# pnnl/nmrfit

Measured on NVIDIA B200. Metric: voigt_objective_evals_per_s, higher is better.
Workload: dtype f64

## Files before the change

### nmrfit_b200/csrc/cabi.cu

```cuda
#include <cuda_runtime.h>
#include <algorithm>
#include <cmath>
#include <atomic>
#include <cstdio>
#include <cstdlib>
#include <cstring>
#include <new>
#include <string>
#include <vector>
#include "../../include/nmrfit_b200.h"
#include "nmrfit_internal.h"

namespace nmrfit {
std::atomic<long long> g_launches{0};
void count_launches(int n) { g_launches.fetch_add(n, std::memory_order_relaxed); }
}

using namespace nmrfit;

namespace {

thread_local std::string t_error;

int fail(int code, const std::string& msg) {
    t_error = msg;
    return code;
}

int fail_cuda(cudaError_t e, const char* where) {
    t_error = std::string(where) + ": " + cudaGetErrorName(e) + " (" + cudaGetErrorString(e) + ")";
    return NMRFIT_ERR_CUDA;
}

#define CK(call)                                              \
    do {                                                      \
        cudaError_t _e = (call);                              \
        if (_e != cudaSuccess) return fail_cuda(_e, #call);   \
    } while (0)

template <typename T>
struct DevBuf {
    T* ptr = nullptr;
    size_t cap = 0;
    cudaError_t reserve(size_t n) {
        if (n <= cap) return cudaSuccess;
        if (ptr) cudaFree(ptr);
        ptr = nullptr;
        cap = 0;
        cudaError_t e = cudaMalloc(&ptr, n * sizeof(T));
        if (e == cudaSuccess) cap = n;
        return e;
    }
    void release() {
        if (ptr) cudaFree(ptr);
        ptr = nullptr;
        cap = 0;
    }
};

bool is_device_pointer(const void* p) {
    cudaPointerAttributes at;
    if (cudaPointerGetAttributes(&at, p) != cudaSuccess) {
        cudaGetLastError();
        return false;
    }
    return at.type == cudaMemoryTypeDevice || at.type == cudaMemoryTypeManaged;
}

}

constexpr int kShadowSpectra = 4;

struct nmrfit_ctx {
    int device = 0, B = 0, N = 0, P = 0, D = 0, precision = 0;
    DevBuf<double> spec;
    std::vector<char> spec_set;
    std::vector<std::vector<double>> shadow;
    DevBuf<double> grid_h;
    std::vector<char> uniform;
    int algorithm = NMRFIT_ALGO_AUTO;
    DevBuf<double> partials, x_stage, f_stage;
    DevBuf<double> prep_coef, prep_part, prep_far, prep_anchor;
    DevBuf<unsigned> prep_mask;
    ObjTune user_tune{0, 0, 0, 0, -1, 0, 0};
    bool swarm = false;
    SwarmState sw{};
    int maxiter = 0, kk = 0, generation = 0;
    DevBuf<double> sx, sv, sp, sfx, sfp, sg, sfg, sbx, sbf, slb, sub, srec, rnd_a, rnd_b;
    DevBuf<int> sstop, sit;
    DevBuf<double> frec_f, frec_x;
    DevBuf<unsigned> fbarrier;
    DevBuf<int> ferror;
    DevBuf<unsigned> mt_state;
    DevBuf<unsigned> mt_words;
    long long mt_elems = 0;
    DevBuf<double> mt_a[2], mt_b[2];
    DevBuf<unsigned> mt_state2, mt_words2;
    cudaStream_t mt_stream = nullptr;
    unsigned* mt_host = nullptr;
    int mt_flip = 0, mt_pending = 0;
    DevBuf<double> fin_scratch;
    DevBuf<unsigned> fin_tickets;
    void* peer_win = nullptr;
    size_t peer_rec_bytes = 0;
    int peer_ranks = 0, peer_rank = 0;
    bool peers_ready = false;
    std::vector<void*> peer_opened;
    DevBuf<double*> peer_recs_dev;
    DevBuf<long long*> peer_tok_dev;
    DevBuf<int> peer_err;
    long long epoch = 0;
    double peer_timeout_ms = 20000.0;
    DevBuf<double> wscratch, wbounds;
    cudaStream_t pipe[2] = {nullptr, nullptr};
    double* h_f = nullptr;
    size_t h_f_cap = 0;
    int far_cells = 0;
    int fused_mode = NMRFIT_FUSED_AUTO;
    DevBuf<long long> ftiming;
    bool fused_timing = false;
    long long fused_launches = 0;
    int* h_flags = nullptr;
    bool profiling = false;
    std::vector<cudaEvent_t> prof_events;
    size_t prof_used = 0;
};

struct nmrfit_phase {
    int device = 0, B = 0, N = 0;
    DevBuf<double> u, v, cands, out;
    DevBuf<int> ok;
};

struct nmrfit_peaks {
    int device = 0, B = 0, N = 0, upsample = 100, max_peaks = 0;
    long long M = 0;
    int nblk = 0;
    DevBuf<double> w, u, uu, us, bmax, base, uu_at, pk_h, sg;
    DevBuf<long long> maxima, pk_i, cross, probe_idx;
    DevBuf<int> n_maxima, n_pk;
    DevBuf<char> out;
    DevBuf<double> probe_out;
    bool ran = false;
};

namespace {

bool axis_is_uniform(const double* hw, int N, double* grid) {
    double h = 0.0, big = 0.0;
    bool uni = N >= 2;
    if (uni) {
        h = (hw[N - 1] - hw[0]) / (double)(N - 1);
        big = std::max(std::fabs(hw[0]), std::fabs(hw[N - 1]));
        const double tol = 4.0 * 2.220446049250313e-16 * big;
        uni = std::isfinite(h) && h != 0.0 && std::isfinite(big);
        for (int i = 0; uni && i < N; ++i) uni = std::fabs(hw[i] - std::fma((double)i, h, hw[0])) <= tol;
    }
    grid[0] = h;
    grid[1] = 2.220446049250313e-16 * big;
    return uni;
}

bool use_uniform(const nmrfit_ctx* c, int fit_im) {
    if (c->algorithm == NMRFIT_ALGO_GENERAL) return false;
    if (fit_im == NMRFIT_IM_SUM || (fit_im == NMRFIT_IM_REFERENCE && c->precision != NMRFIT_FP64)) return false;
    for (char u : c->uniform)
        if (!u) return false;
    return true;
}

int ctx_cells(const nmrfit_ctx* c, int r) { return c->far_cells ? c->far_cells : far_cells_per_region(c->N, r); }

ObjTune pick_tune(const nmrfit_ctx* c, int S, bool uni) {
    ObjTune t;
    if (uni) {
        if (c->N >= 2048) { t.threads = 256; t.r = 8; }
        else { t.threads = 128; t.r = 4; }
    } else {
        if (c->N >= 8192) { t.threads = 256; t.r = 4; }
        else if (c->N >= 1024) { t.threads = 128; t.r = 4; }
        else { t.threads = 128; t.r = 2; }
    }
    t.tb = 6;
    if (c->user_tune.threads) t.threads = c->user_tune.threads;
    if (c->user_tune.r) t.r = c->user_tune.r;
    if (c->user_tune.tb == -1) t.tb = 0;
    else if (c->user_tune.tb > 0) t.tb = c->user_tune.tb;
    int n_tiles = (c->N + t.threads * t.r - 1) / (t.threads * t.r);
    long long ctas1 = (long long)n_tiles * S * c->B;
    int sp = (int)std::max<long long>(1, std::min<long long>(16, ctas1 / (148 * 4)));
    sp = std::min(sp, std::max(1, S));
    if (c->user_tune.sp > 0) sp = std::min(c->user_tune.sp, std::max(1, S));
    t.sp = sp;
    t.variant = 0;
    t.stages = 0;
    t.occ = 3;
    const long long particle_tiles = (long long)((c->N + t.threads * t.r - 1) / (t.threads * t.r)) * S * c->B;
    const bool enough = particle_tiles >= 8192 || c->user_tune.variant == 1;
    if (uni && c->precision == NMRFIT_FP64 && c->user_tune.variant != 0 && t.tb == 6 && enough) {
        t.variant = 1;
        t.occ = c->user_tune.occ == 3 ? 3 : 2;
        const size_t budget = (t.occ == 2 ? 112 : 74) * 1024;
        auto fit_sp = [&](int stg) {
            t.stages = stg;
            int spg = 0;
            for (int cand = 1; cand <= 16; ++cand) {
                t.sp = cand;
                if (objective_stream_smem_bytes(c->P, t, ctx_cells(c, t.r)) <= budget) spg = cand;
            }
            return spg;
        };
        int stg = c->user_tune.stages > 0 ? c->user_tune.stages : 3;
        int spg = fit_sp(stg);
        if (c->user_tune.stages == 0 && spg < 6) {
            const int spg2 = fit_sp(2);
            if (spg2 > spg) { stg = 2; spg = spg2; }
        }
        t.stages = stg;
        t.sp = std::max(1, spg);
        bool fits = true;
        if (c->user_tune.sp > 0) {
            t.sp = c->user_tune.sp;
            if (objective_stream_smem_bytes(c->P, t, ctx_cells(c, t.r)) > 200 * 1024 && c->user_tune.stages == 0) t.stages = 2;
            fits = objective_stream_smem_bytes(c->P, t, ctx_cells(c, t.r)) <= 200 * 1024;
        }
        if (fits) {
            t.sp = std::min(t.sp, std::max(1, S));
            return t;
        }
        t.variant = 0;
        t.stages = 0;
        t.occ = 3;
    }
    const bool f32 = c->precision == NMRFIT_FP32;
    auto uni_bytes = [&]() { return f32 ? objective_f32_smem_bytes(c->P, t) : objective_uniform_smem_bytes(c->P, t, ctx_cells(c, t.r)); };
    while (t.sp > 1 && (uni ? uni_bytes() : objective_smem_bytes(c->P, t, 2)) > 200 * 1024)
        t.sp /= 2;
    if (uni && c->user_tune.sp <= 0)
        while (t.sp > 4 && uni_bytes() > 74 * 1024) t.sp -= 1;
    return t;
}

int check_ctx(const nmrfit_ctx* c) {
    if (!c) return fail(NMRFIT_ERR_ARG, "ctx is NULL");
    return NMRFIT_OK;
}

int run_objective(nmrfit_ctx* c, const double* x_dev, int S, int fit_im, double* f_dev, const int* frozen,
                  cudaStream_t st, const MoveArgs* mv = nullptr, int* tiles_out = nullptr, int* nsum_out = nullptr,
                  int* nw_out = nullptr, size_t slot0 = 0, size_t slots_total = 0, const double* x_in = nullptr) {
    for (int b = 0; b < c->B; ++b)
        if (!c->spec_set[b]) return fail(NMRFIT_ERR_STATE, "spectrum " + std::to_string(b) + " was never set");
    if (fit_im < 0 || fit_im > 2) return fail(NMRFIT_ERR_ARG, "fit_im must be 0, 1 or 2");
    const bool uni = use_uniform(c, fit_im);
    if (c->algorithm == NMRFIT_ALGO_UNIFORM && !uni)
        return fail(NMRFIT_ERR_STATE, "the uniform-axis kernel needs uniformly spaced w in every spectrum and fit_im off");
    if (c->precision == NMRFIT_FP32 && fit_im != NMRFIT_REAL_ONLY)
        return fail(NMRFIT_ERR_ARG, "fit_im is not available in FP32 mode (the Kramers-Kronig term runs in FP64 only)");
    ObjTune t = pick_tune(c, S, uni);
    if (uni && c->precision == NMRFIT_FP32 && t.r == 16) t.r = 8;
    if (uni ? (t.r != 4 && t.r != 8 && t.r != 16) : (t.r != 2 && t.r != 4 && t.r != 8))
        return fail(NMRFIT_ERR_ARG, uni ? "points_per_thread must be 4, 8 or 16 for the uniform-axis kernel"
                                        : "points_per_thread must be 2, 4 or 8 for the general kernel");
    int n_tiles = objective_tiles(c->N, t);
    const size_t part_per = (size_t)n_tiles * 2 * (t.variant == 1 ? t.threads / 32 : 1);
    CK(c->partials.reserve(std::max((size_t)c->B * S, slots_total) * part_per));
    ObjArgs a{};
    const int sub = (uni && c->precision == NMRFIT_FP64) ? ctx_cells(c, t.r) : 1;
    if (uni) {
        size_t nc, np, nf, na, nm;
        int pad = 0;
        objective_uniform_prep_sizes(c->N, c->P, t, sub, &nc, &np, &nf, &na, &nm, &pad);
        const size_t slots = std::max((size_t)c->B * S, slots_total) + pad;
        CK(c->prep_coef.reserve(slots * nc));
        CK(c->prep_part.reserve(slots * np));
        CK(c->prep_far.reserve(slots * nf));
        CK(c->prep_anchor.reserve(slots * na));
        CK(c->prep_mask.reserve(slots * nm));
        a.prep_coef = c->prep_coef.ptr + slot0 * nc; a.prep_part = c->prep_part.ptr + slot0 * np;
        a.prep_far = c->prep_far.ptr + slot0 * nf; a.prep_anchor = c->prep_anchor.ptr + slot0 * na;
        a.prep_mask = c->prep_mask.ptr + slot0 * nm;
    }
    a.spec = c->spec.ptr;
    a.x = x_dev;
    a.x_in = x_in;
    a.partials = c->partials.ptr + slot0 * part_per;
    a.frozen = frozen;
    a.grid_h = c->grid_h.ptr;
    a.N = c->N; a.P = c->P; a.S = S; a.kk = fit_im; a.sp = t.sp; a.sub = sub;
    cudaEvent_t ev0 = nullptr, evm = nullptr, ev1 = nullptr;
    if (c->profiling) {
        if (c->prof_used + 3 > c->prof_events.size()) {
            for (int k = 0; k < 3; ++k) {
                cudaEvent_t ev;
                CK(cudaEventCreate(&ev));
                c->prof_events.push_back(ev);
            }
        }
        ev0 = c->prof_events[c->prof_used];
        evm = c->prof_events[c->prof_used + 1];
        ev1 = c->prof_events[c->prof_used + 2];
        c->prof_used += 3;
    }
    const bool two_pass = uni && c->precision == NMRFIT_FP64;
    if (evm && !two_pass) {
        CK(cudaEventRecord(ev0, st));
        CK(cudaEventRecord(evm, st));
        ev0 = nullptr;
    }
    const bool move_in_prepare = mv && uni && c->precision == NMRFIT_FP64;
    if (mv && !move_in_prepare) {
        cudaError_t em = launch_swarm_move(mv->s, mv->rp, mv->rg, mv->generation, st);
        if (em != cudaSuccess) return fail_cuda(em, "swarm move");
    }
    if (nsum_out) *nsum_out = c->precision == NMRFIT_FP32 ? 1 : (fit_im ? 2 : 1);
    if (nw_out) *nw_out = 1;
    cudaError_t e = c->precision == NMRFIT_FP32 ? launch_objective_f32(a, t, c->B, f_dev, uni, st, ev0, ev1, tiles_out)
                    : uni ? launch_objective_uniform(a, t, c->B, f_dev, st, ev0, ev1, move_in_prepare ? mv : nullptr, tiles_out, evm, nw_out)
                          : launch_objective(a, t, c->B, f_dev, st, ev0, ev1, tiles_out);
    if (e != cudaSuccess) return fail_cuda(e, "objective launch");
    return NMRFIT_OK;
}

int stage(const double* src, size_t n, DevBuf<double>& buf, cudaStream_t st, const double** out) {
    if (!src) { *out = nullptr; return NMRFIT_OK; }
    if (is_device_pointer(src)) { *out = src; return NMRFIT_OK; }
    CK(buf.reserve(n));
    CK(cudaMemcpyAsync(buf.ptr, src, n * sizeof(double), cudaMemcpyHostToDevice, st));
    *out = buf.ptr;
    return NMRFIT_OK;
}

int fused_setup(nmrfit_ctx* c, int n_gen, const double* rp_d, const double* rg_d, FusedArgs* a, FusedPlan* plan) {
    plan->ok = false;
    if (c->fused_mode == NMRFIT_FUSED_OFF) return NMRFIT_OK;
    if (c->precision != NMRFIT_FP64 || c->kk != NMRFIT_REAL_ONLY || !use_uniform(c, NMRFIT_REAL_ONLY)) return NMRFIT_OK;
    const SwarmState& s = c->sw;
    ObjTune t = pick_tune(c, s.S, true);
    *a = FusedArgs{};
    a->s = s;
    a->spec = c->spec.ptr;
    a->grid_h = c->grid_h.ptr;
    a->rp = rp_d;
    a->rg = rg_d;
    a->N = c->N; a->P = c->P;
    a->n_vtiles = objective_tiles(c->N, t);
    a->vw = t.threads / 32;
    a->sub = ctx_cells(c, t.r);
    a->n_gen = n_gen;
    a->gen0 = c->generation + 1;
    a->maxiter = c->maxiter;
    cudaError_t e = swarm_fused_plan(*a, c->D, s.B, s.S, t, c->device, c->fused_mode == NMRFIT_FUSED_REQUIRE, plan);
    if (e != cudaSuccess) return fail_cuda(e, "fused swarm plan");
    if (!plan->ok) return NMRFIT_OK;
    CK(c->frec_f.reserve(2 * (size_t)s.B * s.S));
    CK(c->frec_x.reserve(2 * (size_t)s.B * s.S * s.D));
    CK(c->fbarrier.reserve(s.B));
    if (!c->ferror.ptr) {
        CK(c->ferror.reserve(1));
        CK(cudaMemset(c->ferror.ptr, 0, sizeof(int)));
    }
    a->error = c->ferror.ptr;
    a->max_wait_ns = 10LL * 1000 * 1000 * 1000;
    a->rec_f = c->frec_f.ptr;
    a->rec_x = c->frec_x.ptr;
    a->barrier = c->fbarrier.ptr;
    a->timing = c->fused_timing ? c->ftiming.ptr : nullptr;
    return NMRFIT_OK;
}

PeerArgs make_peer_args(const nmrfit_ctx* c) {
    PeerArgs pa{};
    pa.recs = c->peer_recs_dev.ptr;
    pa.tokens = c->peer_tok_dev.ptr;
    pa.n_ranks = c->peer_ranks;
    pa.rank = c->peer_rank;
    pa.token = (c->epoch << 32) | (long long)c->generation;
    pa.max_wait_ns = (long long)(c->peer_timeout_ms * 1e6);
    pa.error = c->peer_err.ptr;
    return pa;
}

int swarm_generation(nmrfit_ctx* c, bool move, const double* rp_d, const double* rg_d, int commit, cudaStream_t st) {
    SwarmState& s = c->sw;
    if (commit == 2 && !c->peers_ready) return fail(NMRFIT_ERR_STATE, "nmrfit_pso_peer_open has not been called");
    const PeerArgs pa = commit == 2 ? make_peer_args(c) : PeerArgs{};
    MoveArgs mv{s, rp_d, rg_d, c->generation};
    int n_tiles = 0, nsum = 1, nw = 1;
    if (int rc = run_objective(c, s.x, s.S, c->kk, nullptr, move ? s.stop : nullptr, st, move ? &mv : nullptr, &n_tiles, &nsum,
                               &nw))
        return rc;
    cudaError_t e = launch_swarm_finish(s, c->partials.ptr, n_tiles, nsum, c->N, s.rec, c->fin_scratch.ptr,
                                        c->fin_tickets.ptr, commit, c->maxiter, st, nw, commit == 2 ? &pa : nullptr);
    if (e != cudaSuccess) return fail_cuda(e, "swarm finish");
    return NMRFIT_OK;
}

}

extern "C" {

int nmrfit_abi_version(void) { return NMRFIT_ABI_VERSION; }

const char* nmrfit_last_error(void) { return t_error.c_str(); }

int nmrfit_device_count(int* count) {
    if (!count) return fail(NMRFIT_ERR_ARG, "count is NULL");
    CK(cudaGetDeviceCount(count));
    return NMRFIT_OK;
}

long long nmrfit_launch_count(void) { return g_launches.load(); }

int nmrfit_ctx_create(nmrfit_ctx** out, int device, int n_spectra, int n_points, int n_peaks, int precision) {
    if (!out) return fail(NMRFIT_ERR_ARG, "out is NULL");
    *out = nullptr;
    if (n_spectra < 1 || n_points < 1 || n_peaks < 1) return fail(NMRFIT_ERR_ARG, "n_spectra, n_points, n_peaks must be >= 1");
    if (n_peaks > 256) return fail(NMRFIT_ERR_ARG, "n_peaks > 256 is not supported");
    if (precision != NMRFIT_FP64 && precision != NMRFIT_FP32) return fail(NMRFIT_ERR_ARG, "unknown precision");
    int ndev = 0;
    CK(cudaGetDeviceCount(&ndev));
    if (device < 0 || device >= ndev) return fail(NMRFIT_ERR_ARG, "no such CUDA device");
    CK(cudaSetDevice(device));
    nmrfit_ctx* c = new (std::nothrow) nmrfit_ctx();
    if (!c) return fail(NMRFIT_ERR_NOMEM, "out of host memory");
    c->device = device; c->B = n_spectra; c->N = n_points; c->P = n_peaks; c->D = 4 + 3 * n_peaks;
    c->precision = precision;
    c->spec_set.assign(n_spectra, 0);
    c->uniform.assign(n_spectra, 0);
    cudaError_t e = c->spec.reserve((size_t)n_spectra * 4 * n_points);
    if (e == cudaSuccess) e = c->grid_h.reserve(2 * (size_t)n_spectra);
    if (e == cudaSuccess) e = cudaMallocHost(&c->h_flags, sizeof(int) * 2 * n_spectra);
    if (e != cudaSuccess) {
        nmrfit_ctx_destroy(c);
        return fail_cuda(e, "ctx allocation");
    }
    *out = c;
    return NMRFIT_OK;
}

void nmrfit_ctx_destroy(nmrfit_ctx* c) {
    if (!c) return;
    cudaSetDevice(c->device);
    c->prep_mask.release();
    for (DevBuf<double>* b : {&c->prep_coef, &c->prep_part, &c->prep_far, &c->prep_anchor, &c->spec, &c->grid_h, &c->partials, &c->x_stage, &c->f_stage, &c->sx, &c->sv, &c->sp, &c->sfx,
                              &c->sfp, &c->sg, &c->sfg, &c->sbx, &c->sbf, &c->slb, &c->sub, &c->srec, &c->rnd_a,
                              &c->rnd_b})
        b->release();
    c->sstop.release();
    c->sit.release();
    c->frec_f.release();
    c->frec_x.release();
    c->fbarrier.release();
    c->ferror.release();
    c->mt_state.release();
    for (int k = 0; k < 2; ++k) { c->mt_a[k].release(); c->mt_b[k].release(); }
    c->mt_state2.release();
    c->mt_words2.release();
    if (c->mt_stream) cudaStreamDestroy(c->mt_stream);
    if (c->mt_host) cudaFreeHost(c->mt_host);
    c->mt_words.release();
    c->ftiming.release();
    for (void* p : c->peer_opened) cudaIpcCloseMemHandle(p);
    if (c->peer_win) cudaFree(c->peer_win);
    c->peer_recs_dev.release();
    c->peer_tok_dev.release();
    c->peer_err.release();
    c->wscratch.release();
    c->fin_scratch.release();
    c->fin_tickets.release();
    c->wbounds.release();
    for (int k = 0; k < 2; ++k)
        if (c->pipe[k]) cudaStreamDestroy(c->pipe[k]);
    if (c->h_f) cudaFreeHost(c->h_f);
    if (c->h_flags) cudaFreeHost(c->h_flags);
    for (cudaEvent_t ev : c->prof_events) cudaEventDestroy(ev);
    delete c;
}

int nmrfit_ctx_set_spectrum(nmrfit_ctx* c, int b, const double* w, const double* u, const double* v,
                            const double* weights) {
    if (int r = check_ctx(c)) return r;
    if (b < 0 || b >= c->B) return fail(NMRFIT_ERR_ARG, "spectrum index out of range");
    if (!w || !u || !v || !weights) return fail(NMRFIT_ERR_ARG, "w, u, v, weights must be non-NULL");
    CK(cudaSetDevice(c->device));
    double* dst = c->spec.ptr + (size_t)b * 4 * c->N;
    const double* src[4] = {w, u, v, weights};
    const bool host_src = !is_device_pointer(w) && !is_device_pointer(u) && !is_device_pointer(v) && !is_device_pointer(weights);
    const bool shadowed = c->B <= kShadowSpectra && host_src;
    const size_t plane = sizeof(double) * (size_t)c->N;
    if (shadowed) {
        if (c->shadow.empty()) c->shadow.resize(c->B);
        std::vector<double>& sh = c->shadow[b];
        if (c->spec_set[b] && sh.size() == 4 * (size_t)c->N) {
            bool same = true;
            for (int k = 0; same && k < 4; ++k) same = std::memcmp(sh.data() + (size_t)k * c->N, src[k], plane) == 0;
            if (same) return NMRFIT_OK;
        }
        sh.resize(4 * (size_t)c->N);
        for (int k = 0; k < 4; ++k) std::memcpy(sh.data() + (size_t)k * c->N, src[k], plane);
    } else if (!c->shadow.empty()) {
        c->shadow[b].clear();
    }
    for (int k = 0; k < 4; ++k)
        CK(cudaMemcpy(dst + (size_t)k * c->N, src[k], sizeof(double) * c->N, cudaMemcpyDefault));
    std::vector<double> hw;
    const double* wh = w;
    if (is_device_pointer(w)) {
        hw.resize(c->N);
        CK(cudaMemcpy(hw.data(), dst, sizeof(double) * c->N, cudaMemcpyDeviceToHost));
        wh = hw.data();
// ... 1171 lines not shown
```

### nmrfit_b200/csrc/objective_stream.cu

```cuda
#include <cuda_runtime.h>
#include <algorithm>
#include <cstdint>
#include "nmrfit_internal.h"
#include "nmrfit_math.cuh"
#include "uniform_common.cuh"
#include "uniform_eval.cuh"

namespace nmrfit {

namespace {

template <int TB> struct ExpTabS { static __device__ __forceinline__ const double* src() { return nullptr; } };
template <> struct ExpTabS<6> { static __device__ __forceinline__ const double* src() { return NMRFIT_EXP2_TAB6; } };

struct StreamSmem {
    int tab, uv, wt, wfirst, bars, tickets, slot0, slot, coef, part, far, anchor, mask, mw, total;
    __host__ __device__ StreamSmem(int spg, int stages, int P, int threads, int R, int TB, int sub) {
        const int nw = threads / 32;
        mw = (P + 31) / 32;
        int o = 0;
        tab = o;     o += TB ? (1 << TB) : 0;
        uv = o;      o += threads * R * 2;
        wt = o;      o += threads * R;
        wfirst = o;  o += threads;
        bars = o;    o += stages;
        tickets = o; o += (stages + 1) / 2 * 2;
        if (o & 1) ++o;
        slot0 = o;
        int q = 0;
        coef = q;    q += spg * P * 8;
        part = q;    q += spg * kPartDoubles;
        far = q;     q += spg * nw * sub * kFarPoly;
        anchor = q;  q += spg * nw * 2;
        mask = q;    q += ((spg * nw * mask_words_per_region(P, sub) + 3) / 4) * 2;
        slot = q;
        total = slot0 + stages * slot;
    }
};

__device__ __forceinline__ void fence_proxy_async_smem() { asm volatile("fence.proxy.async.shared::cta;" ::: "memory"); }

template <int THREADS, int R, int TB, int KK, int OCC, int SUB>
__global__ void __launch_bounds__(THREADS, (R <= 8 ? OCC * 256 : 512) / THREADS)
objective_stream_kernel(ObjArgs a) {
    constexpr int NSUM = KK ? 2 : 1;
    constexpr int NW = THREADS / 32;
    extern __shared__ __align__(16) double smem[];
    const int b = blockIdx.z;
    if (a.frozen && a.frozen[b]) return;
    const int tid = threadIdx.x, lane = tid & 31, warp = tid >> 5;
    const int P = a.P, N = a.N, D = 4 + 3 * P, SPG = a.sp, ST = a.stages;
    const int n_tiles = a.n_tiles, tile = blockIdx.y, NRP = n_tiles * NW;
    const StreamSmem L(SPG, ST, P, THREADS, R, TB, SUB);
    const int MW = L.mw;
    double* tab = smem + L.tab;
    double2* suv = reinterpret_cast<double2*>(smem + L.uv);
    double* swt = smem + L.wt;
    double* swf = smem + L.wfirst;
    uint64_t* bars = reinterpret_cast<uint64_t*>(smem + L.bars);
    int* tickets = reinterpret_cast<int*>(smem + L.tickets);
    double* slots = smem + L.slot0;

    const int n_groups = (a.S + SPG - 1) / SPG;
    const int g_lo = blockIdx.x * a.gpc, g_hi = min(n_groups, g_lo + a.gpc);
    const int my_groups = g_hi - g_lo;
    if (my_groups <= 0) return;

    const int tile0 = tile * (THREADS * R);
    const double* sw = a.spec + (size_t)b * 4 * N;
    const double h = a.grid_h[2 * b], w_ulp = a.grid_h[2 * b + 1];
    const size_t pb = (size_t)b * a.S;
    const size_t tb_ = ((size_t)b * n_tiles + tile) * a.S;

    const uint32_t b_coef = SPG * P * 8 * 8, b_part = SPG * kPartDoubles * 8, b_far = SPG * NW * SUB * kFarPoly * 8;
    const int MWR = mask_words_per_region(P, SUB);
    const uint32_t b_anchor = SPG * NW * 2 * 8, b_mask = SPG * NW * MWR * 4;
    auto fill = [&](int g) {
        const int sl = g % ST;
        double* dst = slots + (size_t)sl * L.slot;
        const size_t q0 = (size_t)(g_lo + g) * SPG;
        uint64_t* bar = bars + sl;
        mbar_expect_tx(bar, b_coef + b_part + b_far + b_anchor + b_mask);
        bulk_g2s(dst + L.coef, a.prep_coef + (pb + q0) * P * 8, b_coef, bar);
        bulk_g2s(dst + L.part, a.prep_part + (pb + q0) * kPartDoubles, b_part, bar);
        bulk_g2s(dst + L.far, a.prep_far + (tb_ + q0) * NW * SUB * kFarPoly, b_far, bar);
        bulk_g2s(dst + L.anchor, a.prep_anchor + (tb_ + q0) * NW * 2, b_anchor, bar);
        bulk_g2s(dst + L.mask, a.prep_mask + (tb_ + q0) * NW * MWR, b_mask, bar);
    };

    if (tid == 0) {
        for (int s = 0; s < ST; ++s) {
            mbar_init(bars + s, 1);
            tickets[s] = 0;
        }
        asm volatile("fence.mbarrier_init.release.cluster;" ::: "memory");
        for (int g = 0; g < min(ST, my_groups); ++g) fill(g);
    }
    for (int e = tid; e < THREADS * R; e += THREADS) {
        const int i = tile0 + e;
        const bool ok = i < N;
        const int t = e / R, j = e % R;
        const double wgt = ok ? sw[3 * N + i] : 0.0;
        suv[j * THREADS + t] = stage_point(ok ? sw[N + i] : 0.0, ok ? sw[2 * N + i] : 0.0, wgt);
        swt[j * THREADS + t] = wgt;
    }
    {
        const int i_first = tile0 + tid * R;
        swf[tid] = i_first < N ? sw[i_first] : fma((double)i_first, h, sw[0]);
    }
    if (TB) {
        const double* src = ExpTabS<TB>::src();
        for (int i = tid; i < (1 << TB); i += THREADS) tab[i] = src[i];
    }
    constexpr double H = 16.0 * R;
    const double xi0 = cell_xi0<R>(lane, SUB);
    const LaneCell lcell = lane_cell(lane, SUB, P);
    const double inv_H = (double)SUB / H;
    __syncthreads();

    const int s_coef = P * 8, s_far = NW * SUB * kFarPoly, s_mask = NW * MWR;
    const size_t s_out = (size_t)n_tiles * NW * NSUM;
    int sl = 0;
    uint32_t phase = 0;
    for (int g = 0; g < my_groups; ++g) {
        const double* slot = slots + (size_t)sl * L.slot;
        const size_t q0 = (size_t)(g_lo + g) * SPG;
        const int nsp = min(SPG, a.S - (int)q0);
        const int rw = (warp + g) & (NW - 1);
        const int t = rw * 32 + lane;
        const int i_first = tile0 + t * R;
        const double w_first = swf[t];
        const double* cf = slot + L.coef;
        const double* pt = slot + L.part;
        const double* fc = slot + L.far + rw * SUB * kFarPoly;
        const double2* an = reinterpret_cast<const double2*>(slot + L.anchor) + rw;
        const unsigned* mk = reinterpret_cast<const unsigned*>(slot + L.mask) + rw * MWR;
        const double* xs = a.x + (pb + q0) * D;
        double* out = a.partials + (((pb + q0) * n_tiles + tile) * NW + rw) * NSUM;
        mbar_wait(bars + sl, phase);
        for (int sp = 0; sp < nsp; ++sp) {
            double ssi = 0.0;
            const double ss = eval_region<R, TB, KK, false, SUB>(cf, pt, mk, fc, *an, MW, P, lane, lcell, w_first, xi0, inv_H, suv,
                                                            swt, t, THREADS, tab, xs, sw + i_first, N - i_first, h, w_ulp,
                                                            &ssi);
            if (lane == 0) {
                out[0] = ss;
                if (KK) out[1] = ssi;
            }
            cf += s_coef; pt += kPartDoubles; fc += s_far; an += NW; mk += s_mask; xs += D; out += s_out;
        }
        __syncwarp();
        if (lane == 0) {
            __threadfence_block();
            const int old = atomicAdd(tickets + sl, 1);
            if (old == NW - 1) {
                tickets[sl] = 0;
                __threadfence_block();
                if (g + ST < my_groups) {
                    fence_proxy_async_smem();
                    fill(g + ST);
                }
            }
        }
        if (++sl == ST) { sl = 0; phase ^= 1u; }
    }
    (void)NRP;
}

template <int THREADS, int R, int TB, int KK, int OCC, int SUB>
cudaError_t launch_sub(const ObjArgs& a, int B, cudaStream_t st) {
    static bool attr_set[NMRFIT_MAX_DEVICES] = {};
    StreamSmem L(a.sp, a.stages, a.P, THREADS, R, TB, a.sub);
    const size_t bytes = (size_t)L.total * sizeof(double);
    int dev = 0;
    cudaGetDevice(&dev);
    if (!attr_set[dev % NMRFIT_MAX_DEVICES]) {
        cudaError_t e = cudaFuncSetAttribute(objective_stream_kernel<THREADS, R, TB, KK, OCC, SUB>,
                                             cudaFuncAttributeMaxDynamicSharedMemorySize, 200 * 1024);
        if (e != cudaSuccess) return e;
        attr_set[dev % NMRFIT_MAX_DEVICES] = true;
    }
    const int n_groups = (a.S + a.sp - 1) / a.sp;
    dim3 grid((n_groups + a.gpc - 1) / a.gpc, a.n_tiles, B);
    objective_stream_kernel<THREADS, R, TB, KK, OCC, SUB><<<grid, THREADS, bytes, st>>>(a);
    return cudaGetLastError();
}

template <int THREADS, int R, int TB, int KK, int OCC>
cudaError_t launch_occ(const ObjArgs& a, int B, cudaStream_t st) {
    switch (a.sub) {
        case 1: return launch_sub<THREADS, R, TB, KK, OCC, 1>(a, B, st);
        case 2: return launch_sub<THREADS, R, TB, KK, OCC, 2>(a, B, st);
        case 4: return launch_sub<THREADS, R, TB, KK, OCC, 4>(a, B, st);
        default: return cudaErrorInvalidValue;
    }
}

template <int THREADS, int R, int TB, int KK>
cudaError_t launch_one(const ObjArgs& a, int B, cudaStream_t st) {
    return a.occ == 2 ? launch_occ<THREADS, R, TB, KK, 2>(a, B, st) : launch_occ<THREADS, R, TB, KK, 3>(a, B, st);
}

template <int THREADS, int R>
cudaError_t launch_tb(const ObjArgs& a, int tb, int B, cudaStream_t st) {
    switch (tb) {
        case 6: return a.kk ? launch_one<THREADS, R, 6, 1>(a, B, st) : launch_one<THREADS, R, 6, 0>(a, B, st);
        default: return cudaErrorInvalidValue;
    }
}

}

size_t objective_stream_smem_bytes(int P, const ObjTune& t, int sub) {
    return (size_t)StreamSmem(t.sp, t.stages, P, t.threads, t.r, t.tb, sub).total * sizeof(double);
}

cudaError_t launch_objective_stream(const ObjArgs& a, const ObjTune& t, int B, cudaStream_t st) {
    if (t.threads == 128 && t.r == 4) return launch_tb<128, 4>(a, t.tb, B, st);
    if (t.threads == 128 && t.r == 8) return launch_tb<128, 8>(a, t.tb, B, st);
    if (t.threads == 128 && t.r == 16) return launch_tb<128, 16>(a, t.tb, B, st);
    if (t.threads == 256 && t.r == 4) return launch_tb<256, 4>(a, t.tb, B, st);
    if (t.threads == 256 && t.r == 8) return launch_tb<256, 8>(a, t.tb, B, st);
    if (t.threads == 256 && t.r == 16) return launch_tb<256, 16>(a, t.tb, B, st);
    return cudaErrorInvalidValue;
}

}
```

### nmrfit_b200/csrc/uniform_eval.cuh

```cuda
#pragma once
#include <cuda_runtime.h>
#include "nmrfit_math.cuh"
#include "uniform_common.cuh"

namespace nmrfit {

__host__ __device__ inline int mask_words_per_region(int P, int sub) { return (sub == 1 ? 1 : sub + 1) * ((P + 31) / 32 + 1); }

constexpr int kPairDoubles = kFarTerms + 1;
constexpr int kTableItems = 33;

template <int R>
__device__ __forceinline__ void prep_item_coef(const double* __restrict__ xs, int k, double h, double w_ulp,
                                               double* __restrict__ cs, double* __restrict__ coef_out,
                                               double* __restrict__ farpk, int sub, int P, double* __restrict__ part) {
    if (k == 0) part[66] = (double)P * xs[3];
    SpanCoef c = make_span_coef(xs[2], xs[4 + 3 * k], xs[5 + 3 * k], xs[6 + 3 * k], h, w_ulp, R);
    if (c.exact) c = null_span_coef();
    double* o = cs + k * 8;
    o[0] = c.loc; o[1] = c.kL; o[2] = c.kG; o[3] = c.aL; o[4] = c.aG; o[5] = c.dT; o[6] = c.thr; o[7] = c.c2;
    const FarPeak f = make_far_peak(c, 0.5 * (double)(32 * R / sub));
    double* q = farpk + k * 4;
    q[0] = f.A; q[1] = f.A2; q[2] = f.A2x; q[3] = f.reach;
    if (coef_out) {
        double* g = coef_out + k * 8;
#pragma unroll
        for (int i = 0; i < 8; ++i) g[i] = o[i];
    }
}

template <int R>
__device__ __forceinline__ double prep_item_angle(const double* __restrict__ xs, int it, int N, double inv_N) {
    if (it < 32) return (xs[1] * (double)(it * R)) * inv_N;
    if (it == 32) return xs[1] * inv_N;
    const int ra = it - kTableItems;
    return (long long)ra * 32 * R < N ? fma(xs[1] * (double)(ra * 32 * R), inv_N, xs[0]) : 0.0;
}

__device__ __forceinline__ int fast_div(int e, int d, float inv) {
    int q = __float2int_rz(__int2float_rn(e) * inv);
    const int r = e - q * d;
    q += (r >= d) - (r < 0);
    return q;
}

__device__ __forceinline__ void prep_item_exact_count(const double* __restrict__ cs, int P, double* __restrict__ part) {
    int n = 0;
    for (int k = 0; k < P; ++k) n += cs[k * 8 + 6] < 0.0;
    part[67] = (double)n;
}

template <int R>
__device__ __forceinline__ void prep_item_pair(const double* __restrict__ cs, const double* __restrict__ farpk,
                                               const double* __restrict__ sw, double h, int N,
                                               int sub, long long ic, int k, double* __restrict__ pr) {
    const int cell_pts = 32 * R / sub;
    double kind = -1.0;
    if (ic < N) {
        const double* o = cs + k * 8;
        if (!(o[6] < 0.0)) {
            const double* q = farpk + k * 4;
            FarPeak f;
            f.A = q[0]; f.A2 = q[1]; f.A2x = q[2]; f.reach = q[3];
            const double w_c = fma(0.5 * (double)(cell_pts - 1), h, sw[ic]);
            double v[kFarTerms];
            kind = (double)far_terms_pre(w_c - o[0], o[1], o[2], f, v);
#pragma unroll
            for (int n = 0; n < kFarTerms; ++n) pr[1 + n] = v[n];
        }
    }
    pr[0] = kind;
}

template <int R>
__device__ __forceinline__ void prep_item_cell(bool ok, const double* __restrict__ cs, const double* __restrict__ farpk,
                                               const double* __restrict__ sw, double h, int N, int P, int sub, long long ic, int ci,
                                               const double* __restrict__ pairs_row, double* __restrict__ far_dst,
                                               unsigned* __restrict__ mask_region) {
    const int MW = (P + 31) / 32;
    const int cell_pts = 32 * R / sub;
    double C[kFarTerms];
#pragma unroll
    for (int n = 0; n < kFarTerms; ++n) C[n] = 0.0;
    unsigned any_far = 0;
    unsigned* mk = mask_region + (sub == 1 ? 0 : 1 + ci) * (MW + 1);
    const bool live = ok && ic < N;
    const double w_c = (live && !pairs_row) ? fma(0.5 * (double)(cell_pts - 1), h, sw[ic]) : 0.0;
    for (int wd = 0; wd < MW; ++wd) {
        unsigned m = 0;
        if (live) {
            const int kend = min(P, wd * 32 + 32);
            for (int k = wd * 32; k < kend; ++k) {
                if (pairs_row) {
                    const double* pr = pairs_row + (size_t)k * kPairDoubles;
                    const int kind = (int)pr[0];
                    if (kind < 0) continue;
                    if (kind == kFarNear) { m |= 1u << (k & 31); continue; }
                    any_far = 1u;
                    if (kind == kFarSeries) {
                        double v[kFarTerms];
#pragma unroll
                        for (int n = 0; n < kFarTerms; ++n) v[n] = pr[1 + n];
                        far_add(cs[k * 8 + 3], v, C);
                    }
                } else {
                    const double* o = cs + k * 8;
                    if (o[6] < 0.0) continue;
                    const double2 c01 = *reinterpret_cast<const double2*>(o);
                    const double2 c23 = *reinterpret_cast<const double2*>(o + 2);
                    const double2 f01 = *reinterpret_cast<const double2*>(farpk + k * 4);
                    const double2 f23 = *reinterpret_cast<const double2*>(farpk + k * 4 + 2);
                    FarPeak f;
                    f.A = f01.x; f.A2 = f01.y; f.A2x = f23.x; f.reach = f23.y;
                    double v[kFarTerms];
                    const int kind = far_terms_pre(w_c - c01.x, c01.y, c23.x, f, v);
                    if (kind == kFarNear) { m |= 1u << (k & 31); continue; }
                    any_far = 1u;
                    if (kind == kFarSeries) far_add(c23.y, v, C);
                }
            }
        }
        if (ok) mk[wd] = m;
        if (sub > 1) {
            unsigned mu = m;
            for (int o = 1; o < sub; o <<= 1) mu |= __shfl_xor_sync(0xffffffffu, mu, o);
            if (ok && ci == 0) mask_region[wd] = mu;
        }
    }
    if (ok) mk[MW] = any_far;
    if (sub > 1) {
        unsigned fu = any_far;
        for (int o = 1; o < sub; o <<= 1) fu |= __shfl_xor_sync(0xffffffffu, fu, o);
        if (ok && ci == 0) mask_region[MW] = fu;
    }
    if (ok) {
        far_economise(C);
#pragma unroll
        for (int n = 0; n < kFarPoly; n += 2) *reinterpret_cast<double2*>(far_dst + n) = make_double2(C[n], C[n + 1]);
    }
}

template <int R>
__device__ __forceinline__ void prepare_particle(const double* __restrict__ xs, const double* __restrict__ sw, double h,
                                                 double w_ulp, int N, int P, int NR, int NRP, int tid, int nthreads,
                                                 double* __restrict__ cs, double* __restrict__ coef_out,
                                                 double* __restrict__ part, double* __restrict__ far,
                                                 double* __restrict__ anchor, unsigned* __restrict__ mask,
                                                 double* __restrict__ farpk, double* __restrict__ pairs = nullptr,
                                                 int r_lo = 0, int r_hi = -1, int sub = 1) {
    if (r_hi < 0) r_hi = NRP;
    const int nr = r_hi - r_lo, nc = nr * sub;
    const int cell_pts = 32 * R / sub;
    const int MWR = mask_words_per_region(P, sub);
    (void)NR;
    for (int k = tid; k < P; k += nthreads) prep_item_coef<R>(xs, k, h, w_ulp, cs, coef_out, farpk, sub, P, part);
    const double inv_N = 1.0 / (double)N;
    for (int e = nthreads - 1 - tid; e < kTableItems + nr; e += nthreads) {
        double sn, cn;
        sincos(prep_item_angle<R>(xs, e < kTableItems ? e : e + r_lo, N, inv_N), &sn, &cn);
        double* dst = e < kTableItems ? part + 2 * e : anchor + 2 * (e - kTableItems);
        dst[0] = cn;
        dst[1] = sn;
    }
    __syncthreads();
    if (tid == nthreads - 1) prep_item_exact_count(cs, P, part);
    if (pairs) {
        for (int pi = tid; pi < nc * P; pi += nthreads) {
            const int cl = pi / P, k = pi - cl * P;
            prep_item_pair<R>(cs, farpk, sw, h, N, sub, ((long long)r_lo * sub + cl) * cell_pts, k,
                              pairs + (size_t)pi * kPairDoubles);
        }
        __syncthreads();
    }
    for (int base = tid & ~31; base < nc; base += nthreads) {
        const int cl = base + (tid & 31);
        const bool ok = cl < nc;
        const int rl = cl / sub, ci = cl - rl * sub;
        prep_item_cell<R>(ok, cs, farpk, sw, h, N, P, sub, ((long long)r_lo * sub + cl) * cell_pts, ci,
                          pairs ? pairs + (size_t)cl * P * kPairDoubles : nullptr, far + (size_t)cl * kFarPoly,
                          mask + (size_t)rl * MWR);
    }
}

__device__ __forceinline__ double2 stage_point(double u, double v, double wt) {
    return make_double2(__dmul_rn(wt, u), __dmul_rn(wt, v));
}
__device__ __forceinline__ int stage_slot_uv(int t, int j, int stride) { return j * stride + (t ^ j); }
__device__ __forceinline__ int stage_slot_wt(int t, int j, int stride) { return j * stride + (t ^ (2 * j)); }

struct LaneCell { int mk_off, fc_off, mirror; };
__device__ __forceinline__ LaneCell lane_cell(int lane, int sub, int P) {
    const int cell = (lane * sub) >> 5, MW = (P + 31) / 32;
    LaneCell lc;
    lc.mk_off = sub == 1 ? 0 : (1 + cell) * (MW + 1);
    lc.fc_off = cell * kFarPoly;
    lc.mirror = 32 / sub - 1;
    return lc;
}

template <int R, int TB, int KK = 0, bool SWZ = true, int SUBT = 0>
__device__ __forceinline__ double eval_region(const double* __restrict__ cf, const double* __restrict__ pt,
                                              const unsigned* __restrict__ mk, const double* __restrict__ fc,
                                              const double2 ew, int MW, int P, int lane, const LaneCell lc, double w_first, double xi0,
                                              double inv_H, const double2* __restrict__ suv, const double* __restrict__ swt,
                                              int t, int stride, const double* __restrict__ tab,
                                              const double* __restrict__ xs, const double* __restrict__ sw_first,
                                              int n_valid, double h, double w_ulp, double* ss_im = nullptr) {
    const unsigned* mkc = mk + lc.mk_off;
    double acc[R];
    const double py = pt[66];
    {
        const double* fcc = fc + lc.fc_off;
        double C[kFarPoly];
#pragma unroll
        for (int n = 0; n < kFarPoly; n += 2) {
            const double2 t2 = *reinterpret_cast<const double2*>(fcc + n);
            C[n] = t2.x; C[n + 1] = t2.y;
        }
        C[0] += py;
        double mir[R / 2];
        far_init_half<R>(C, xi0, inv_H, acc, mir);
#pragma unroll
        for (int j = 0; j < R / 2; ++j) acc[R - 1 - j] = __shfl_xor_sync(0xffffffffu, mir[j], SUBT ? 32 / SUBT - 1 : lc.mirror);
    }
    for (int wd = 0; wd < MW; ++wd) {
        const unsigned mine = mkc[wd];
        for (unsigned m = mk[wd]; m; m &= m - 1) {
            const int kb = __ffs(m) - 1;
            const int k = wd * 32 + kb;
            const double2 c01 = *reinterpret_cast<const double2*>(cf + k * 8);
            const double2 c23 = *reinterpret_cast<const double2*>(cf + k * 8 + 2);
            const double2 c45 = *reinterpret_cast<const double2*>(cf + k * 8 + 4);
            const double2 c67 = *reinterpret_cast<const double2*>(cf + k * 8 + 6);
            SpanCoef c;
            c.loc = c01.x; c.kL = c01.y; c.kG = c23.x; c.aL = c23.y;
            c.aG = c45.x; c.dT = c45.y; c.thr = c67.x; c.c2 = c67.y;
            if ((SUBT ? SUBT == 1 : lc.mk_off == 0) || ((mine >> kb) & 1u)) peak_span<R, TB>(w_first - c.loc, c, tab, acc);
        }
    }
    if (pt[67] != 0.0) {
        for (int k = 0; k < P; ++k) {
            if (!(cf[k * 8 + 6] < 0.0)) continue;
            const SpanCoef c = make_span_coef(xs[2], xs[4 + 3 * k], xs[5 + 3 * k], xs[6 + 3 * k], h, w_ulp, R);
            peak_exact<R, TB>(sw_first, n_valid, w_first, h, c, tab, acc);
        }
    }
    const double2 el = *reinterpret_cast<const double2*>(pt + 2 * lane);
    const double cd = pt[64], sd = pt[65];
    double cr = fma(ew.x, el.x, -(ew.y * el.y));
    double ci = fma(ew.y, el.x, ew.x * el.y);
    double ss = 0.0, ssi = 0.0;
    double kloc = 0.0, kkL = 0.0, kkG = 0.0, kaL = 0.0, kaG = 0.0;
    bool kexact = false;
    if (KK) {
        const double* cl = cf + (P - 1) * 8;
        kexact = cl[6] < 0.0;
        if (kexact) {
            const int k = P - 1;
            const SpanCoef c = make_span_coef(xs[2], xs[4 + 3 * k], xs[5 + 3 * k], xs[6 + 3 * k], h, w_ulp, R);
            kloc = c.loc; kkL = c.kL; kkG = c.kG; kaL = c.aL; kaG = c.aG * kTwoOverSqrtPi;
        } else {
            kloc = cl[0]; kkL = cl[1]; kkG = cl[2]; kaL = cl[3]; kaG = cl[4] * kTwoOverSqrtPi;
        }
    }
    const double2* puv = suv + t;
    const double* pwt = swt + t;
#pragma unroll
    for (int j = 0; j < R; ++j) {
        const double2 uv = SWZ ? suv[stage_slot_uv(t, j, stride)] : puv[j * stride];
        const double wt = SWZ ? swt[stage_slot_wt(t, j, stride)] : pwt[j * stride];
        const double res = fma(uv.x, cr, -fma(uv.y, ci, wt * acc[j]));
        ss = fma(res, res, ss);
        if (KK) {
            const double idat = fma(uv.x, ci, uv.y * cr);
            const double wj = (kexact && j < n_valid) ? sw_first[j] : (j == 0 ? w_first : fma((double)j, h, w_first));
            const double d = wj - kloc;
            const double tt = d * kkL;
            const double rq = rcp_pos(fma(tt, tt, 1.0));
            const double daw = dawson(d * kkG, NMRFIT_DAW_TAB, NMRFIT_DAW_TAIL);
            const double ifit = fma(kaL * tt, rq, kaG * daw);
            const double ri = fma(-wt, ifit, idat);
            ssi = fma(ri, ri, ssi);
        }
        if (j + 1 < R) {
            const double c2 = fma(cr, cd, -(ci * sd));
            ci = fma(ci, cd, cr * sd);
            cr = c2;
        }
    }
#pragma unroll
    for (int o = 16; o > 0; o >>= 1) {
        ss += __shfl_xor_sync(0xffffffffu, ss, o);
        if (KK) ssi += __shfl_xor_sync(0xffffffffu, ssi, o);
    }
    if (KK) *ss_im = ssi;
    return ss;
}

template <int R>
__device__ __forceinline__ double cell_xi0(int lane, int sub) {
    const int lpc = 32 / sub;
    const double H = 0.5 * (double)(lpc * R);
    return ((double)((lane % lpc) * R) - 0.5 * (double)(lpc * R - 1)) / H;
}

}
```

Baseline: 70.87 million.

## Evaluate SUB spectra per warp pass with lane groups covering each far-field cell

Adds a multi-spectrum path for the OCC=2, SUB>1, non-KK stream kernel. Each warp splits into SUB lane groups, and each group evaluates a different parameter set by looping over all far-field cells of the region. Near-peak masks are OR-reduced across the warp so per-cell peak work converges, and the reduction shrinks to the lane group. The host tuner now picks spectra-per-group counts divisible by the cell count and uses a slightly larger shared-memory budget. The goal is to cut divergence from cell-specific peak masks and redundant per-spectrum overhead, at the cost of extra per-lane serial loops and masked tail work.

```diff
diff --git a/nmrfit_b200/csrc/cabi.cu b/nmrfit_b200/csrc/cabi.cu
--- a/nmrfit_b200/csrc/cabi.cu
+++ b/nmrfit_b200/csrc/cabi.cu
@@ -200,13 +200,15 @@
     if (uni && c->precision == NMRFIT_FP64 && c->user_tune.variant != 0 && t.tb == 6 && enough) {
         t.variant = 1;
         t.occ = c->user_tune.occ == 3 ? 3 : 2;
-        const size_t budget = (t.occ == 2 ? 112 : 74) * 1024;
+        const size_t budget = t.occ == 2 ? 115712 : 74 * 1024;
+        const int cells = ctx_cells(c, t.r), per_warp = t.occ == 2 ? cells : 1;
         auto fit_sp = [&](int stg) {
             t.stages = stg;
             int spg = 0;
             for (int cand = 1; cand <= 16; ++cand) {
                 t.sp = cand;
-                if (objective_stream_smem_bytes(c->P, t, ctx_cells(c, t.r)) <= budget) spg = cand;
+                if (objective_stream_smem_bytes(c->P, t, cells) <= budget && (cand < per_warp || cand % per_warp == 0))
+                    spg = cand;
             }
             return spg;
         };
diff --git a/nmrfit_b200/csrc/objective_stream.cu b/nmrfit_b200/csrc/objective_stream.cu
--- a/nmrfit_b200/csrc/objective_stream.cu
+++ b/nmrfit_b200/csrc/objective_stream.cu
@@ -45,6 +45,7 @@
 objective_stream_kernel(ObjArgs a) {
     constexpr int NSUM = KK ? 2 : 1;
     constexpr int NW = THREADS / 32;
+    constexpr bool MULTI = SUB > 1 && !KK && OCC == 2;
     extern __shared__ __align__(16) double smem[];
     const int b = blockIdx.z;
     if (a.frozen && a.frozen[b]) return;
@@ -138,7 +139,17 @@
         const double* xs = a.x + (pb + q0) * D;
         double* out = a.partials + (((pb + q0) * n_tiles + tile) * NW + rw) * NSUM;
         mbar_wait(bars + sl, phase);
-        for (int sp = 0; sp < nsp; ++sp) {
+        if constexpr (MULTI) {
+            constexpr int LPC = 32 / SUB;
+            const int q = lane / LPC;
+            for (int sp0 = 0; sp0 < nsp; sp0 += SUB) {
+                const int sp = min(sp0 + q, nsp - 1);
+                const double ss = eval_region_multi<R, TB, SUB>(
+                    cf + sp * s_coef, pt + sp * kPartDoubles, mk + sp * s_mask, fc + sp * s_far, an[sp * NW], MW, P, lane,
+                    xi0, inv_H, suv, swt, swf, rw * 32, THREADS, tab, xs + (size_t)sp * D, sw + tile0, N - tile0, h, w_ulp);
+                if ((lane & (LPC - 1)) == 0 && sp0 + q < nsp) out[sp * s_out] = ss;
+            }
+        } else for (int sp = 0; sp < nsp; ++sp) {
             double ssi = 0.0;
             const double ss = eval_region<R, TB, KK, false, SUB>(cf, pt, mk, fc, *an, MW, P, lane, lcell, w_first, xi0, inv_H, suv,
                                                             swt, t, THREADS, tab, xs, sw + i_first, N - i_first, h, w_ulp,
diff --git a/nmrfit_b200/csrc/uniform_eval.cuh b/nmrfit_b200/csrc/uniform_eval.cuh
--- a/nmrfit_b200/csrc/uniform_eval.cuh
+++ b/nmrfit_b200/csrc/uniform_eval.cuh
@@ -198,46 +198,40 @@
     return lc;
 }
 
-template <int R, int TB, int KK = 0, bool SWZ = true, int SUBT = 0>
-__device__ __forceinline__ double eval_region(const double* __restrict__ cf, const double* __restrict__ pt,
-                                              const unsigned* __restrict__ mk, const double* __restrict__ fc,
-                                              const double2 ew, int MW, int P, int lane, const LaneCell lc, double w_first, double xi0,
-                                              double inv_H, const double2* __restrict__ suv, const double* __restrict__ swt,
-                                              int t, int stride, const double* __restrict__ tab,
-                                              const double* __restrict__ xs, const double* __restrict__ sw_first,
-                                              int n_valid, double h, double w_ulp, double* ss_im = nullptr) {
-    const unsigned* mkc = mk + lc.mk_off;
-    double acc[R];
-    const double py = pt[66];
-    {
-        const double* fcc = fc + lc.fc_off;
-        double C[kFarPoly];
-#pragma unroll
-        for (int n = 0; n < kFarPoly; n += 2) {
-            const double2 t2 = *reinterpret_cast<const double2*>(fcc + n);
-            C[n] = t2.x; C[n + 1] = t2.y;
-        }
-        C[0] += py;
-        double mir[R / 2];
-        far_init_half<R>(C, xi0, inv_H, acc, mir);
-#pragma unroll
-        for (int j = 0; j < R / 2; ++j) acc[R - 1 - j] = __shfl_xor_sync(0xffffffffu, mir[j], SUBT ? 32 / SUBT - 1 : lc.mirror);
-    }
-    for (int wd = 0; wd < MW; ++wd) {
-        const unsigned mine = mkc[wd];
-        for (unsigned m = mk[wd]; m; m &= m - 1) {
-            const int kb = __ffs(m) - 1;
-            const int k = wd * 32 + kb;
-            const double2 c01 = *reinterpret_cast<const double2*>(cf + k * 8);
-            const double2 c23 = *reinterpret_cast<const double2*>(cf + k * 8 + 2);
-            const double2 c45 = *reinterpret_cast<const double2*>(cf + k * 8 + 4);
-            const double2 c67 = *reinterpret_cast<const double2*>(cf + k * 8 + 6);
-            SpanCoef c;
-            c.loc = c01.x; c.kL = c01.y; c.kG = c23.x; c.aL = c23.y;
-            c.aG = c45.x; c.dT = c45.y; c.thr = c67.x; c.c2 = c67.y;
-            if ((SUBT ? SUBT == 1 : lc.mk_off == 0) || ((mine >> kb) & 1u)) peak_span<R, TB>(w_first - c.loc, c, tab, acc);
-        }
-    }
+template <int R>
+__device__ __forceinline__ void lane_far_start(const double* __restrict__ fcc, double py, double xi0, double inv_H,
+                                               int mirror, double (&acc)[R]) {
+    double C[kFarPoly];
+#pragma unroll
+    for (int n = 0; n < kFarPoly; n += 2) {
+        const double2 t2 = *reinterpret_cast<const double2*>(fcc + n);
+        C[n] = t2.x; C[n + 1] = t2.y;
+    }
+    C[0] += py;
+    double mir[R / 2];
+    far_init_half<R>(C, xi0, inv_H, acc, mir);
+#pragma unroll
+    for (int j = 0; j < R / 2; ++j) acc[R - 1 - j] = __shfl_xor_sync(0xffffffffu, mir[j], mirror);
+}
+
+template <int R, int TB>
+__device__ __forceinline__ void lane_near_peak(const double* __restrict__ cf, int k, double w_first,
+                                               const double* __restrict__ tab, double (&acc)[R]) {
+    const double2 c01 = *reinterpret_cast<const double2*>(cf + k * 8);
+    const double2 c23 = *reinterpret_cast<const double2*>(cf + k * 8 + 2);
+    const double2 c45 = *reinterpret_cast<const double2*>(cf + k * 8 + 4);
+    const double2 c67 = *reinterpret_cast<const double2*>(cf + k * 8 + 6);
+    SpanCoef c;
+    c.loc = c01.x; c.kL = c01.y; c.kG = c23.x; c.aL = c23.y;
+    c.aG = c45.x; c.dT = c45.y; c.thr = c67.x; c.c2 = c67.y;
+    peak_span<R, TB>(w_first - c.loc, c, tab, acc);
+}
+
+template <int R, int TB>
+__device__ __forceinline__ void lane_exact_peaks(const double* __restrict__ cf, const double* __restrict__ pt, int P,
+                                                 const double* __restrict__ xs, const double* __restrict__ sw_first,
+                                                 int n_valid, double w_first, double h, double w_ulp,
+                                                 const double* __restrict__ tab, double (&acc)[R]) {
     if (pt[67] != 0.0) {
         for (int k = 0; k < P; ++k) {
             if (!(cf[k * 8 + 6] < 0.0)) continue;
@@ -245,7 +239,16 @@
             peak_exact<R, TB>(sw_first, n_valid, w_first, h, c, tab, acc);
         }
     }
-    const double2 el = *reinterpret_cast<const double2*>(pt + 2 * lane);
+}
+
+template <int R, int KK, bool SWZ>
+__device__ __forceinline__ double lane_residual(const double (&acc)[R], const double* __restrict__ cf,
+                                                const double* __restrict__ pt, int P, const double2 ew, int lf,
+                                                const double2* __restrict__ suv, const double* __restrict__ swt, int t,
+                                                int stride, const double* __restrict__ xs,
+                                                const double* __restrict__ sw_first, int n_valid, double w_first,
+                                                double h, double w_ulp, double* ssi_out) {
+    const double2 el = *reinterpret_cast<const double2*>(pt + 2 * lf);
     const double cd = pt[64], sd = pt[65];
     double cr = fma(ew.x, el.x, -(ew.y * el.y));
     double ci = fma(ew.y, el.x, ew.x * el.y);
@@ -288,12 +291,77 @@
             cr = c2;
         }
     }
+    if (KK) *ssi_out = ssi;
+    return ss;
+}
+
+template <int R, int TB, int KK = 0, bool SWZ = true, int SUBT = 0>
+__device__ __forceinline__ double eval_region(const double* __restrict__ cf, const double* __restrict__ pt,
+                                              const unsigned* __restrict__ mk, const double* __restrict__ fc,
+                                              const double2 ew, int MW, int P, int lane, const LaneCell lc, double w_first, double xi0,
+                                              double inv_H, const double2* __restrict__ suv, const double* __restrict__ swt,
+                                              int t, int stride, const double* __restrict__ tab,
+                                              const double* __restrict__ xs, const double* __restrict__ sw_first,
+                                              int n_valid, double h, double w_ulp, double* ss_im = nullptr) {
+    const unsigned* mkc = mk + lc.mk_off;
+    double acc[R];
+    lane_far_start<R>(fc + lc.fc_off, pt[66], xi0, inv_H, SUBT ? 32 / SUBT - 1 : lc.mirror, acc);
+    for (int wd = 0; wd < MW; ++wd) {
+        const unsigned mine = mkc[wd];
+        for (unsigned m = mk[wd]; m; m &= m - 1) {
+            const int kb = __ffs(m) - 1;
+            if ((SUBT ? SUBT == 1 : lc.mk_off == 0) || ((mine >> kb) & 1u)) lane_near_peak<R, TB>(cf, wd * 32 + kb, w_first, tab, acc);
+        }
+    }
+    lane_exact_peaks<R, TB>(cf, pt, P, xs, sw_first, n_valid, w_first, h, w_ulp, tab, acc);
+    double ssi = 0.0;
+    double ss = lane_residual<R, KK, SWZ>(acc, cf, pt, P, ew, lane, suv, swt, t, stride, xs, sw_first, n_valid, w_first,
+                                          h, w_ulp, &ssi);
 #pragma unroll
     for (int o = 16; o > 0; o >>= 1) {
         ss += __shfl_xor_sync(0xffffffffu, ss, o);
         if (KK) ssi += __shfl_xor_sync(0xffffffffu, ssi, o);
     }
     if (KK) *ss_im = ssi;
+    return ss;
+}
+
+template <int R, int TB, int SUB>
+__device__ __forceinline__ double eval_region_multi(const double* __restrict__ cf, const double* __restrict__ pt,
+                                                    const unsigned* __restrict__ mk, const double* __restrict__ fc,
+                                                    const double2 ew, int MW, int P, int lane, double xi0, double inv_H,
+                                                    const double2* __restrict__ suv, const double* __restrict__ swt,
+                                                    const double* __restrict__ swf, int t0, int stride,
+                                                    const double* __restrict__ tab, const double* __restrict__ xs,
+                                                    const double* __restrict__ sw_tile, int n_tile, double h, double w_ulp) {
+    static_assert(SUB == 2 || SUB == 4, "one pass per far-field cell of the region");
+    constexpr int LPC = 32 / SUB;
+    const int i = lane & (LPC - 1);
+    const double py = pt[66];
+    double se = 0.0, so = 0.0;
+#pragma unroll 1
+    for (int c = 0; c < SUB; ++c) {
+        const int lf = c * LPC + i, t = t0 + lf;
+        const double w_first = swf[t];
+        double acc[R];
+        lane_far_start<R>(fc + c * kFarPoly, py, xi0, inv_H, LPC - 1, acc);
+        const unsigned* mkc = mk + (1 + c) * (MW + 1);
+        for (int wd = 0; wd < MW; ++wd) {
+            const unsigned mine = mkc[wd];
+            for (unsigned m = __reduce_or_sync(0xffffffffu, mine); m; m &= m - 1) {
+                const int kb = __ffs(m) - 1;
+                if ((mine >> kb) & 1u) lane_near_peak<R, TB>(cf, wd * 32 + kb, w_first, tab, acc);
+            }
+        }
+        lane_exact_peaks<R, TB>(cf, pt, P, xs, sw_tile + t * R, n_tile - t * R, w_first, h, w_ulp, tab, acc);
+        const double s = lane_residual<R, 0, false>(acc, cf, pt, P, ew, lf, suv, swt, t, stride, xs, sw_tile + t * R,
+                                                    n_tile - t * R, w_first, h, w_ulp, nullptr);
+        if (c & 1) so += s;
+        else se += s;
+    }
+    double ss = se + so;
+#pragma unroll
+    for (int o = LPC / 2; o > 0; o >>= 1) ss += __shfl_xor_sync(0xffffffffu, ss, o);
     return ss;
 }
 
```

New measurement: 76.13 million, median of 6. 1.07x the previous value.
